# hpc4cmb/flacarray

Hardware: AMD Instinct MI355X
Metric: Msamples/s encode+decode, 4096ch x 1Msamp int32 (higher is better)
Workload: dtype int32

## Files before the change

### flacarray_amd/csrc/encode_fused.hpp

```cpp
#pragma once
#include "encode_kernels.hpp"
#include "quantize_kernels.hpp"

namespace fa {

constexpr int kFSmpWords = 65 * 32;
#ifndef FA_F_SCANW
#define FA_F_SCANW 4
#endif
#ifndef FA_F_RING
#define FA_F_RING 1024
#endif
constexpr int kFRingWords = FA_F_RING;
constexpr int kFRingMask = kFRingWords - 1;
constexpr int kFRingBlocks = kFRingWords / 64;
constexpr int kFRowBlocks = 12;
static_assert(kFRingBlocks - kFRowBlocks - 1 >= 1, "the ring must hold the longest row and a partial block beside what waits to be flushed");
constexpr int kFWaveWords = kFSmpWords + kFRingWords + 4 + 16;
constexpr int kFWaves = 4;
constexpr int kFCrcSlice = 1024;
constexpr int kFCrcXpow = 520;
#ifndef FA_F_SLEEP
#define FA_F_SLEEP 8
#endif
#ifndef FA_F_WBATCH
#define FA_F_WBATCH 4
#endif
#ifndef FA_F_CEIL
#define FA_F_CEIL 1
#endif
#ifndef FA_F_BFLY_N
#define FA_F_BFLY_N 1
#endif
#ifndef FA_F_PARKN
#define FA_F_PARKN 32
#endif
#ifndef FA_F_PARKBLK
#define FA_F_PARKBLK 1
#endif
#ifndef FA_F_PARK
#define FA_F_PARK 1
#endif
#ifndef FA_F_WAVES
#define FA_F_WAVES 3
#endif
constexpr uint32_t kLbSpinLimit = 1u << 22;

struct FusedArgs {
    const int32_t* data;
    const float* f_offsets;
    const float* f_gains;
    int64_t n_stream, stream_size, nframes, total_frames;
    int32_t max_lpc_order, max_porder, precision, pmax_full;
    int32_t tail_bs;
    double escale_full;
    const float* win;
    const uint4* hdr;
    uint8_t* blob;
    int64_t capacity;
    int64_t hb;
    uint32_t* frame_bytes;
    int64_t* frame_abs;
    FrameInfo* info;
    uint32_t* ticket;
    uint32_t* size_pub;
    unsigned long long* off_pub;
    int64_t* total;
    int* err;
    const uint16_t* crc_tab;
    unsigned long long* stamps;
    int64_t* starts;
    int64_t* nbytes;
};

__device__ __forceinline__ int fsmp_unit(int c1, int u) { return 32 * c1 + 4 * (u ^ (c1 & 7)); }
__device__ __forceinline__ int fsmp_idx(int s) {
    const int c1 = (s >> 5) + 1;
    return fsmp_unit(c1, (s >> 2) & 7) + (s & 3);
}

__device__ __forceinline__ int lane_id_opaque() {
    int l;
    asm volatile("v_mbcnt_lo_u32_b32 %0, -1, 0\n\tv_mbcnt_hi_u32_b32 %0, -1, %0" : "=v"(l));
    return l;
}
__device__ __forceinline__ int rice_fold(int r) { return (int)(((uint32_t)r << 1) ^ (uint32_t)(r >> 31)); }
__device__ __forceinline__ int dpp_wave_shr1(int old, int v) { return __builtin_amdgcn_update_dpp(old, v, 0x138, 0xF, 0xF, false); }

__device__ __forceinline__ uint16_t crc16_mulmod(uint16_t a, uint16_t b) {
    uint32_t r = 0;
#pragma unroll
    for (int i = 15; i >= 0; --i) {
        r = (r << 1) ^ ((r & 0x8000u) ? 0x18005u : 0u);
        if ((b >> i) & 1) r ^= a;
    }
    return (uint16_t)r;
}

template <typename T>
__device__ __forceinline__ T lb_load(const T* p) { return __hip_atomic_load(p, __ATOMIC_RELAXED, __HIP_MEMORY_SCOPE_AGENT); }

struct SplitRiceSearch {
    int pred_order, pmax, lane;
    uint32_t TA, TB, S, n, pb, SC, best;
    int M, p, k, bpo, kb;
    bool slot;
    __device__ __forceinline__ void start(uint32_t ta, uint32_t tb, int pred_order_, int pmax_, int lane_) {
        pred_order = pred_order_; pmax = pmax_; lane = lane_;
        TA = wave_incl_scan_u32(ta);
        TB = wave_incl_scan_u32(tb);
    }
    __device__ __forceinline__ void gather() {
        M = (2 << pmax) - 1;
        const int Lp = M - lane;
        slot = (Lp >= 1);
        const int po = slot ? (31 - __clz(Lp)) : 0;
        p = lane - (M + 1 - (2 << po));
        const uint32_t psz = 4096u >> po;
        const int cpp = 128 >> po;
        const bool inB = (po > 0) && (p >= (1 << (po - 1)));
        const int ph = inB ? (p - (1 << (po - 1))) : p;
        int hi_l = (po == 0) ? 63 : ((ph + 1) * cpp - 1);
        int lo_l = (po == 0) ? -1 : (ph * cpp - 1);
        hi_l &= 63;
        const int lo_c = lo_l < 0 ? 0 : (lo_l & 63);
        const uint32_t ah = (uint32_t)__builtin_amdgcn_ds_bpermute(hi_l << 2, (int)TA);
        const uint32_t bh = (uint32_t)__builtin_amdgcn_ds_bpermute(hi_l << 2, (int)TB);
// ... 160 lines not shown
    const int32_t* src = a.data + (s * a.stream_size + f * (int64_t)bs);
    float q_off = 0.0f, q_gain = 0.0f;
    if constexpr (F32IN) { q_off = a.f_offsets[s]; q_gain = a.f_gains[s]; }
    auto load_row = [&](int j) __attribute__((always_inline)) {
        const int4 v = reinterpret_cast<const int4*>(src)[64 * j + lane];
        if constexpr (F32IN)
            return make_int4(quantise_f32(__int_as_float(v.x), q_off, q_gain), quantise_f32(__int_as_float(v.y), q_off, q_gain),
                             quantise_f32(__int_as_float(v.z), q_off, q_gain), quantise_f32(__int_as_float(v.w), q_off, q_gain));
        else
            return v;
    };
    const float* win = a.win;
    const uint4 fhe = a.hdr[f];
    const uint32_t fh_bits = 32u + ((fhe.w >> 8) & 0xFFu) + ((fhe.w >> 16) & 0xFFu) + (fhe.w >> 24) + 8u;

#define FA_IMAGE_ADDRS                                                                  \
    const int ln_ = lane_id_opaque();                                                   \
    const int K = fsmp_unit(ln_ + 1, 0);                                                \
    const int rowbase = fsmp_unit((ln_ >> 3) + 1, ln_ & 7);                             \
    const int hist7 = fsmp_unit(ln_, 7), hist6 = fsmp_unit(ln_, 6), hist5 = fsmp_unit(ln_, 5); \
    (void)K; (void)rowbase; (void)hist7; (void)hist6; (void)hist5
    constexpr int tailA7 = 32 * 64 + 4 * (7 ^ (64 & 7)), tailA6 = 32 * 64 + 4 * (6 ^ (64 & 7)), tailA5 = 32 * 64 + 4 * (5 ^ (64 & 7));

    FA_STAMP_INIT;
#ifdef FA_TIMELINE
    const uint32_t tl_start_ = (uint32_t)__builtin_amdgcn_s_memrealtime();
#endif
    int4 Bv[8];
    uint32_t orv = 0;
    int mn, mx;
    {
        FA_IMAGE_ADDRS;
        int4 hi[8], lo[8];
#pragma unroll
        for (int j = 0; j < 8; ++j) hi[j] = load_row(8 + j);
#pragma unroll
        for (int j = 0; j < 8; ++j) lo[j] = load_row(j);
        if (lane < 32) smp[lane] = 0;
        mn = hi[0].x;
        mx = hi[0].x;
#pragma unroll
        for (int j = 0; j < 8; ++j) {
            orv |= (uint32_t)(hi[j].x | hi[j].y | hi[j].z | hi[j].w);
            mn = min(min(mn, hi[j].x), hi[j].y);
            mn = min(min(mn, hi[j].z), hi[j].w);
            mx = max(max(mx, hi[j].x), hi[j].y);
            mx = max(max(mx, hi[j].z), hi[j].w);
            *reinterpret_cast<int4*>(&smp[rowbase + 256 * j]) = hi[j];
        }
#pragma unroll
        for (int t = 0; t < 8; ++t) Bv[t] = *reinterpret_cast<const int4*>(&smp[K ^ (4 * t)]);
#pragma unroll
        for (int j = 0; j < 8; ++j) {
            orv |= (uint32_t)(lo[j].x | lo[j].y | lo[j].z | lo[j].w);
            mn = min(min(mn, lo[j].x), lo[j].y);
            mn = min(min(mn, lo[j].z), lo[j].w);
            mx = max(max(mx, lo[j].x), lo[j].y);
            mx = max(max(mx, lo[j].z), lo[j].w);
            *reinterpret_cast<int4*>(&smp[rowbase + 256 * j]) = lo[j];
        }
    }
    mn = wave_min_i32(mn);
    mx = wave_max_i32(mx);
    const bool is_const = (mn == mx);
    orv = wave_or_u32(orv);
    const int wasted = orv ? (__ffs((int)orv) - 1) : 0;
    const int bps = 32 - wasted;
    if (__builtin_expect(wasted != 0, 0)) {
        FA_IMAGE_ADDRS;
#pragma unroll
        for (int t = 0; t < 8; ++t) {
            Bv[t].x >>= wasted; Bv[t].y >>= wasted; Bv[t].z >>= wasted; Bv[t].w >>= wasted;
            int4* p = reinterpret_cast<int4*>(&smp[K ^ (4 * t)]);
            int4 v = *p;
            v.x >>= wasted; v.y >>= wasted; v.z >>= wasted; v.w >>= wasted;
            *p = v;
        }
        mn >>= wasted;
        mx >>= wasted;
    }
    const bool narrow = (mn >= -(1 << 24)) && (mx < (1 << 24));
    lds_fence();

    FA_STAMP(0);
    const uint64_t verbatim_bits = 8 + (uint64_t)wasted + (uint64_t)bs * (uint64_t)bps;
    int type = 1;
    int order = 0, porder = 0, shift = 0, precision = 0;
    int kbest = 0;
    bool img_is_residual = false;
    bool win_small_l = false, win_small_f = false;
    int fo = -1;
    int32_t qkeep[MLO];
#pragma unroll
    for (int j = 0; j < MLO; ++j) qkeep[j] = 0;
    const int pmax_geo = a.pmax_full;
    auto pmax_for = [&](int pred_order) __attribute__((always_inline)) {
        int pm = pmax_geo;
        while (pm > 0 && (bs >> pm) <= pred_order) pm--;
        return pm;
    };

    auto hist_b = [&](const int4& own, const int4& tail) __attribute__((always_inline)) {
        int4 h;
        h.x = dpp_wave_shr1(tail.x, own.x);
        h.y = dpp_wave_shr1(tail.y, own.y);
        h.z = dpp_wave_shr1(tail.z, own.z);
        h.w = dpp_wave_shr1(tail.w, own.w);
        return h;
    };

    if (__builtin_expect(is_const, 0)) {
        type = 0;
    } else {
        uint64_t best_bits = verbatim_bits;
        double tot0 = 0.0, tot1 = 0.0, tot2 = 0.0, tot3 = 0.0, tot4 = 0.0;
        double mx0 = 0.0, mx1 = 0.0, mx2 = 0.0, mx3 = 0.0, mx4 = 0.0;
        uint64_t hA0 = 0, hA1 = 0, hA2 = 0, hA3 = 0, hA4 = 0;
        double dA0 = 0.0, dA1 = 0.0, dA2 = 0.0, dA3 = 0.0, dA4 = 0.0;
        if (__builtin_expect(narrow, 1)) {
            FA_IMAGE_ADDRS;
            const uint32_t BIAS = 0x80000000u;
            uint32_t s0 = 0, s1 = 0, s2 = 0, s3 = 0, s4 = 0;
            int p1, pe1, pe2, pe3;
            auto seed = [&](const int4& hh) __attribute__((always_inline)) {
                p1 = hh.w;
                pe1 = hh.w - hh.z;
                pe2 = pe1 - (hh.z - hh.y);
                pe3 = pe2 - ((hh.z - hh.y) - (hh.y - hh.x));
            };
            auto group = [&](auto mask_tag, const int4& xv, int gi0) __attribute__((always_inline)) {
                constexpr bool MASK = decltype(mask_tag)::value;
                const int xs[4] = {xv.x, xv.y, xv.z, xv.w};
#pragma unroll
                for (int e = 0; e < 4; ++e) {
                    const int x = xs[e];
                    const int e1 = x - p1, e2 = e1 - pe1, e3 = e2 - pe2;
                    const uint32_t xb = (uint32_t)x ^ BIAS;
                    const uint32_t n0 = sad_u32(xb, BIAS, s0);
                    const uint32_t n1 = sad_u32(xb, (uint32_t)p1 ^ BIAS, s1);
                    const uint32_t n2 = sad_u32((uint32_t)e1 ^ BIAS, (uint32_t)pe1 ^ BIAS, s2);
                    const uint32_t n3 = sad_u32((uint32_t)e2 ^ BIAS, (uint32_t)pe2 ^ BIAS, s3);
                    const uint32_t n4 = sad_u32((uint32_t)e3 ^ BIAS, (uint32_t)pe3 ^ BIAS, s4);
                    if constexpr (MASK) {
                        const int gi = gi0 + e;
                        s0 = n0;
                        s1 = (gi >= 1) ? n1 : s1;
                        s2 = (gi >= 2) ? n2 : s2;
                        s3 = (gi >= 3) ? n3 : s3;
                        s4 = (gi >= 4) ? n4 : s4;
                    } else {
                        s0 = n0; s1 = n1; s2 = n2; s3 = n3; s4 = n4;
                    }
                    p1 = x; pe1 = e1; pe2 = e2; pe3 = e3;
                }
            };
            uint64_t a0 = 0, a1 = 0, a2 = 0, a3 = 0, a4 = 0;
            auto fold = [&]() __attribute__((always_inline)) {
                a0 += s0; a1 += s1; a2 += s2; a3 += s3; a4 += s4;
                s0 = s1 = s2 = s3 = s4 = 0;
            };
            seed(*reinterpret_cast<const int4*>(&smp[hist7]));
            group(std::true_type{}, *reinterpret_cast<const int4*>(&smp[K]), 32 * lane);
#pragma unroll
            for (int t = 1; t < 4; ++t) group(std::false_type{}, *reinterpret_cast<const int4*>(&smp[K ^ (4 * t)]), 0);
            fold();
#pragma unroll
            for (int t = 4; t < 8; ++t) group(std::false_type{}, *reinterpret_cast<const int4*>(&smp[K ^ (4 * t)]), 0);
            fold();
            hA0 = a0; hA1 = a1; hA2 = a2; hA3 = a3; hA4 = a4;
            seed(hist_b(Bv[7], *reinterpret_cast<const int4*>(&smp[tailA7])));
#pragma unroll
            for (int t = 0; t < 4; ++t) group(std::false_type{}, Bv[t], 0);
            fold();
#pragma unroll
            for (int t = 4; t < 8; ++t) group(std::false_type{}, Bv[t], 0);
            fold();
            tot0 = (double)a0; tot1 = (double)a1; tot2 = (double)a2; tot3 = (double)a3; tot4 = (double)a4;
        } else {
            FA_IMAGE_ADDRS;
            double p1, pe1, pe2, pe3;
            auto seed = [&](const int4& h) __attribute__((always_inline)) {
                p1 = (double)h.w;
                pe1 = (double)h.w - (double)h.z;
                const double e1b = (double)h.z - (double)h.y;
                pe2 = pe1 - e1b;
                const double e2b = e1b - ((double)h.y - (double)h.x);
                pe3 = pe2 - e2b;
            };
            auto group = [&](const int4& xv, int gi0) __attribute__((always_inline)) {
                const int xs[4] = {xv.x, xv.y, xv.z, xv.w};
#pragma unroll
                for (int e = 0; e < 4; ++e) {
                    const int gi = gi0 + e;
                    const double xd = (double)xs[e];
                    const double e1 = xd - p1;
                    const double e2 = e1 - pe1;
                    const double e3 = e2 - pe2;
                    const double e4 = e3 - pe3;
                    const double a0 = fa_fabs(xd);
                    const double a1 = (gi >= 1) ? fa_fabs(e1) : 0.0;
                    const double a2 = (gi >= 2) ? fa_fabs(e2) : 0.0;
                    const double a3 = (gi >= 3) ? fa_fabs(e3) : 0.0;
                    const double a4 = (gi >= 4) ? fa_fabs(e4) : 0.0;
                    tot0 += a0; tot1 += a1; tot2 += a2; tot3 += a3; tot4 += a4;
                    mx0 = __builtin_fmax(mx0, a0);
                    mx1 = __builtin_fmax(mx1, a1);
                    mx2 = __builtin_fmax(mx2, a2);
                    mx3 = __builtin_fmax(mx3, a3);
                    mx4 = __builtin_fmax(mx4, a4);
                    p1 = xd; pe1 = e1; pe2 = e2; pe3 = e3;
                }
            };
            seed(*reinterpret_cast<const int4*>(&smp[hist7]));
#pragma unroll 1
            for (int t = 0; t < 8; ++t) group(*reinterpret_cast<const int4*>(&smp[K ^ (4 * t)]), 32 * lane + 4 * t);
            dA0 = tot0; dA1 = tot1; dA2 = tot2; dA3 = tot3; dA4 = tot4;
            seed(hist_b(Bv[7], *reinterpret_cast<const int4*>(&smp[tailA7])));
#pragma unroll
            for (int t = 0; t < 8; ++t) group(Bv[t], 4096);
        }
        FA_STAMP(1);
        {
            double tsum[5] = {tot0, tot1, tot2, tot3, tot4};
            wave_sum_butterfly_n<5>(tsum);
            const double T0 = tsum[0], T1 = tsum[1], T2 = tsum[2], T3 = tsum[3], T4 = tsum[4];
            double M0 = 0.0, M1 = 0.0, M2 = 0.0, M3 = 0.0, M4 = 0.0;
            if (!narrow) {
                M0 = wave_max_f64(mx0); M1 = wave_max_f64(mx1); M2 = wave_max_f64(mx2); M3 = wave_max_f64(mx3);
                M4 = wave_max_f64(mx4);
            }
            const double lim = 2147483647.0;
            double smallest = 1.8446744073709552e19;
            if (M0 <= lim && T0 < smallest) { fo = 0; smallest = T0; }
            if (M1 <= lim && T1 < smallest) { fo = 1; smallest = T1; }
            if (M2 <= lim && T2 < smallest) { fo = 2; smallest = T2; }
            if (M3 <= lim && T3 < smallest) { fo = 3; smallest = T3; }
            if (M4 <= lim && T4 < smallest) { fo = 4; smallest = T4; }
        }
        uint64_t fixA, fixB;
        if (narrow) {
            const uint64_t tA = (fo == 0) ? hA0 : (fo == 1) ? hA1 : (fo == 2) ? hA2 : (fo == 3) ? hA3 : hA4;
            const double tt = (fo == 0) ? tot0 : (fo == 1) ? tot1 : (fo == 2) ? tot2 : (fo == 3) ? tot3 : tot4;
            fixA = tA;
            fixB = (uint64_t)tt - tA;
        } else {
            const double tA = (fo == 0) ? dA0 : (fo == 1) ? dA1 : (fo == 2) ? dA2 : (fo == 3) ? dA3 : dA4;
            const double tt = (fo == 0) ? tot0 : (fo == 1) ? tot1 : (fo == 2) ? tot2 : (fo == 3) ? tot3 : tot4;
            fixA = (uint64_t)tA;
            fixB = (uint64_t)(tt - tA);
        }
        int po_fix = 0, k_fix = 0;
        const int pmax_fix = pmax_for(fo < 0 ? 0 : fo);
        const bool small_fix = __all((fixA < (1u << 24)) && (fixB < (1u << 24)));
        win_small_f = small_fix;
        const bool fuse_search = fo >= 0 && pmax_fix <= 5 && a.max_lpc_order > 0 && small_fix;
        uint64_t est_fix = 0;
        auto apply_fixed = [&]() __attribute__((always_inline)) {
            if (est_fix < best_bits) {
                best_bits = est_fix;
                type = 2;
                order = fo;
                porder = po_fix;
                kbest = k_fix;
            }
        };
        if (__builtin_expect(fo >= 0 && !fuse_search, 0)) {
            uint64_t rb;
            if (pmax_fix <= 5 && small_fix) {
                SplitRiceSearch fs;
                fs.start((uint32_t)fixA, (uint32_t)fixB, fo, pmax_fix, lane);
                fs.gather(); fs.params(); fs.totals();
#pragma unroll
                for (int o = 5; o >= 0; --o) fs.order(o);
                po_fix = fs.bpo; k_fix = fs.kb; rb = fs.best;
            } else {
                rb = split_rice_search_slow(fixA, fixB, fo, pmax_fix, lane, &po_fix, &k_fix);
            }
            est_fix = 8 + (uint64_t)wasted + (uint64_t)fo * (uint64_t)bps + rb;
            apply_fixed();
        }

        FA_STAMP(2);
        int mlo = a.max_lpc_order;
        if (__builtin_expect(mlo > 0, 1)) {
            FA_IMAGE_ADDRS;
            double acc[MLO + 1];
#pragma unroll
            for (int j = 0; j <= MLO; ++j) acc[j] = 0.0;
            SplitRiceSearch fs;
            if (fuse_search) fs.start((uint32_t)fixA, (uint32_t)fixB, fo, pmax_fix, lane);
            double hist[MLO];
            struct WinV { double w[4]; };
            auto load_win = [&](int i0) __attribute__((always_inline)) {
                const float4 f = *reinterpret_cast<const float4*>(win + i0);
                WinV v;
                v.w[0] = (double)f.x; v.w[1] = (double)f.y; v.w[2] = (double)f.z; v.w[3] = (double)f.w;
                return v;
            };
            auto lag_group = [&](const int4& xv, const WinV& wv) __attribute__((always_inline)) {
                const int xs[4] = {xv.x, xv.y, xv.z, xv.w};
#pragma unroll
                for (int e = 0; e < 4; ++e) {
                    const double d = (double)xs[e] * wv.w[e];
                    acc[0] = __builtin_fma(d, d, acc[0]);
#pragma unroll
                    for (int j = 0; j < MLO; ++j) acc[j + 1] = __builtin_fma(d, hist[j], acc[j + 1]);
#pragma unroll
                    for (int j = MLO - 1; j > 0; --j) hist[j] = hist[j - 1];
                    hist[0] = d;
                }
            };
            auto search_stage = [&](int tt) __attribute__((always_inline)) {
                if (!fuse_search) return;
                if (tt == 1) fs.gather();
                if (tt == 3) fs.params();
                if (tt == 5) fs.totals();
                if (tt >= 7 && tt <= 12) fs.order(12 - tt);
            };
#if FA_F_PARK
            {
                int4* const pk = reinterpret_cast<int4*>(ring) + lane;
#pragma unroll
                for (int t = 0; t < 4; ++t) pk[64 * t] = Bv[4 + t];
            }
#endif
            {
                const int g0 = 32 * lane;
                const int4 h7 = *reinterpret_cast<const int4*>(&smp[hist7]), h6 = *reinterpret_cast<const int4*>(&smp[hist6]);
                const int4 h5 = *reinterpret_cast<const int4*>(&smp[hist5]);
                const int hs[12] = {h7.w, h7.z, h7.y, h7.x, h6.w, h6.z, h6.y, h6.x, h5.w, h5.z, h5.y, h5.x};
#pragma unroll
                for (int j = 0; j < MLO; ++j) {
                    const float wh = (g0 - 1 - j >= 0) ? win[g0 - 1 - j] : 0.0f;
                    hist[j] = (double)hs[j] * (double)wh;
                }
#pragma unroll
                for (int tb = 0; tb < 8; tb += FA_F_WBATCH) {
                    WinV wv[FA_F_WBATCH];
#pragma unroll
                    for (int t = 0; t < FA_F_WBATCH; ++t) wv[t] = load_win(g0 + 4 * (tb + t));
#pragma unroll
                    for (int t = 0; t < FA_F_WBATCH; ++t) {
                        lag_group(*reinterpret_cast<const int4*>(&smp[K ^ (4 * (tb + t))]), wv[t]);
                        search_stage(tb + t);
                    }
                    __builtin_amdgcn_sched_barrier(0);
                }
            }
#if FA_F_PARK
            {
                uint32_t pin = 16u * (uint32_t)lane;
                asm volatile("" : "+v"(pin) : "v"(__double2loint(acc[MLO])));
                const int4* const pk = reinterpret_cast<const int4*>(reinterpret_cast<const char*>(ring) + pin);
#pragma unroll
                for (int t = 0; t < 4; ++t) Bv[4 + t] = pk[64 * t];
            }
#endif
            {
                const int g0 = 2048 + 32 * lane;
                const int4 h7 = hist_b(Bv[7], *reinterpret_cast<const int4*>(&smp[tailA7]));
                const int4 h6 = hist_b(Bv[6], *reinterpret_cast<const int4*>(&smp[tailA6]));
                int4 h5 = make_int4(0, 0, 0, 0);
                if constexpr (MLO > 8) h5 = hist_b(Bv[5], *reinterpret_cast<const int4*>(&smp[tailA5]));
                const int hs[12] = {h7.w, h7.z, h7.y, h7.x, h6.w, h6.z, h6.y, h6.x, h5.w, h5.z, h5.y, h5.x};
#pragma unroll
                for (int j = 0; j < MLO; ++j) hist[j] = (double)hs[j] * (double)win[g0 - 1 - j];
#pragma unroll
                for (int tb = 0; tb < 8; tb += FA_F_WBATCH) {
                    WinV wv[FA_F_WBATCH];
#pragma unroll
                    for (int t = 0; t < FA_F_WBATCH; ++t) wv[t] = load_win(g0 + 4 * (tb + t));
#pragma unroll
                    for (int t = 0; t < FA_F_WBATCH; ++t) {
                        lag_group(Bv[tb + t], wv[t]);
                        search_stage(8 + tb + t);
                    }
                    __builtin_amdgcn_sched_barrier(0);
                }
            }
            FA_STAMP(4);
            if (fuse_search) {
                po_fix = fs.bpo;
                k_fix = fs.kb;
                est_fix = 8 + (uint64_t)wasted + (uint64_t)fo * (uint64_t)bps + (uint64_t)fs.best;
                apply_fixed();
            }
            double autoc[MLO + 1];
#if FA_F_BFLY_N
#pragma unroll
            for (int j = 0; j <= MLO; ++j) autoc[j] = acc[j];
            wave_sum_butterfly_n<MLO + 1>(autoc);
#else
#pragma unroll
            for (int j = 0; j <= MLO; ++j) autoc[j] = wave_sum_butterfly(acc[j]);
#endif

            FA_STAMP(5);
            if (__builtin_expect(autoc[0] != 0.0, 1)) {
                float* coef = reinterpret_cast<float*>(scr);
                double* err = reinterpret_cast<double*>(scr + 160);
                int* meta = reinterpret_cast<int*>(scr + 220);
                if (lane == 0) meta[0] = levinson<MLO>(autoc, mlo, coef, err);
                lds_fence();
                const int usable = meta[0];
                int prec = a.precision;
                int lo;
                {
                    double mybits = 1e300;
                    if (lane < usable) {
                        const double e = err[lane];
                        const double error_scale = a.escale_full;
                        double bpsv;
                        if (e > 0.0) {
                            bpsv = 0.5 * det_log2(error_scale * e);
                            if (!(bpsv >= 0.0)) bpsv = 0.0;
                        } else if (e < 0.0) {
                            bpsv = 1e32;
                        } else {
                            bpsv = 0.0;
                        }
                        mybits = bpsv * (double)(bs - (lane + 1)) + (double)((lane + 1) * (bps + prec));
                    }
                    double bestb = 4294967295.0;
                    int bi = 0;
#pragma unroll
                    for (int o = 0; o < MLO; ++o) {
                        const double b = readlane_f64(mybits, o);
                        if (o < usable && b < bestb) { bestb = b; bi = o; }
                    }
                    lo = bi + 1;
                }
                if (bps <= 17) {
                    const int limp = 32 - bps - ilog2_u64((uint64_t)lo);
                    if (prec > limp) prec = limp;
                }
                int sh = 0;
                int32_t qreg[MLO];
#pragma unroll
                for (int j = 0; j < MLO; ++j) qreg[j] = 0;
                int ok = 0;
                if (prec >= 2) ok = (quantize_coefs_t<MLO>(coef + (lo - 1) * MLO, lo, prec, qreg, &sh) == 0) ? 1 : 0;
                ok = __builtin_amdgcn_readfirstlane(ok);
                sh = __builtin_amdgcn_readfirstlane(sh);
#pragma unroll
                for (int j = 0; j < MLO; ++j) qreg[j] = __builtin_amdgcn_readfirstlane(qreg[j]);
                FA_STAMP(6);
                if (__builtin_expect(ok != 0, 1)) {
                    FA_IMAGE_ADDRS;
                    const double scale = bitsd((uint64_t)(1023 - sh) << 52);
                    double qd[MLO];
#pragma unroll
                    for (int j = 0; j < MLO; ++j) qd[j] = (double)qreg[j] * scale;
                    double tlA = 0.0, tlB = 0.0;
                    double hx[MLO];
                    const int4 a7 = *reinterpret_cast<const int4*>(&smp[hist7]), a6 = *reinterpret_cast<const int4*>(&smp[hist6]);
                    const int4 a5 = *reinterpret_cast<const int4*>(&smp[hist5]);
                    const int4 b7 = hist_b(Bv[7], *reinterpret_cast<const int4*>(&smp[tailA7]));
                    const int4 b6 = hist_b(Bv[6], *reinterpret_cast<const int4*>(&smp[tailA6]));
                    int4 b5 = make_int4(0, 0, 0, 0);
                    if constexpr (MLO > 8) b5 = hist_b(Bv[5], *reinterpret_cast<const int4*>(&smp[tailA5]));
                    lds_fence();
                    auto fold_f64 = [&](double r) __attribute__((always_inline)) {
                        return (int)(uint32_t)__builtin_fabs(__builtin_fma(r, 2.0, 0.5));
                    };
                    auto res_group = [&](auto mask_tag, const int4& xv, int gi0, double& tl) __attribute__((always_inline)) {
                        constexpr bool MASK = decltype(mask_tag)::value;
                        const int xs[4] = {xv.x, xv.y, xv.z, xv.w};
                        int rs[4];
#pragma unroll
                        for (int e = 0; e < 4; ++e) {
                            const double xd = (double)xs[e];
#if FA_F_CEIL
                            double t = xd;
#pragma unroll
                            for (int j = 0; j < MLO; ++j) t = __builtin_fma(-qd[j], hx[j], t);
                            const double r = fa_ceil(t);
#else
                            double sum = 0.0;
#pragma unroll
                            for (int j = 0; j < MLO; ++j) sum = __builtin_fma(qd[j], hx[j], sum);
                            const double pred = fa_floor(sum);
                            const double r = xd - pred;
#endif
                            if constexpr (MASK) {
                                const bool v = (gi0 + e >= lo);
                                tl += v ? fa_fabs(r) : 0.0;
                                rs[e] = v ? fold_f64(r) : xs[e];
                            } else {
                                tl += fa_fabs(r);
                                rs[e] = fold_f64(r);
                            }
#pragma unroll
                            for (int j = MLO - 1; j > 0; --j) hx[j] = hx[j - 1];
                            hx[0] = xd;
                        }
                        return make_int4(rs[0], rs[1], rs[2], rs[3]);
                    };
                    constexpr int kWarmGroups = (MLO + 3) / 4;
                    {
                        const int hs[12] = {a7.w, a7.z, a7.y, a7.x, a6.w, a6.z, a6.y, a6.x, a5.w, a5.z, a5.y, a5.x};
#pragma unroll
                        for (int j = 0; j < MLO; ++j) hx[j] = (double)hs[j];
#pragma unroll
                        for (int t = 0; t < 8; ++t) {
                            int4* px = reinterpret_cast<int4*>(&smp[K ^ (4 * t)]);
                            if (t < kWarmGroups) *px = res_group(std::true_type{}, *px, 32 * lane + 4 * t, tlA);
                            else *px = res_group(std::false_type{}, *px, 0, tlA);
                        }
                    }
                    {
                        const int hs[12] = {b7.w, b7.z, b7.y, b7.x, b6.w, b6.z, b6.y, b6.x, b5.w, b5.z, b5.y, b5.x};
#pragma unroll
                        for (int j = 0; j < MLO; ++j) hx[j] = (double)hs[j];
#pragma unroll
                        for (int t = 0; t < 8; ++t) Bv[t] = res_group(std::false_type{}, Bv[t], 0, tlB);
                    }
                    FA_STAMP(7);
                    img_is_residual = true;
                    const int pmax = pmax_for(lo);
                    int po_l = 0, k_l = 0;
                    uint64_t rbits;
                    const bool small_l = __all((tlA < 16777216.0) && (tlB < 16777216.0));
                    bool lpc_in_range = true;
                    if (__builtin_expect(!small_l, 0)) {
                        bool hit = false;
#pragma unroll 1
                        for (int t = 0; t < 8; ++t) {
                            const int4 ra = *reinterpret_cast<const int4*>(&smp[K ^ (4 * t)]);
                            const int ras[4] = {ra.x, ra.y, ra.z, ra.w};
#pragma unroll
                            for (int e = 0; e < 4; ++e) hit = hit || ((32 * lane + 4 * t + e >= lo) && (uint32_t)ras[e] == 0xffffffffu);
                        }
#pragma unroll
                        for (int t = 0; t < 8; ++t)
                            hit = hit || (uint32_t)Bv[t].x == 0xffffffffu || (uint32_t)Bv[t].y == 0xffffffffu || (uint32_t)Bv[t].z == 0xffffffffu ||
                                  (uint32_t)Bv[t].w == 0xffffffffu;
                        lpc_in_range = !__any(hit);
                    }
                    win_small_l = small_l;
                    if (pmax <= 5 && small_l) {
                        SplitRiceSearch ls;
                        ls.start((uint32_t)tlA, (uint32_t)tlB, lo, pmax, lane);
                        ls.gather(); ls.params(); ls.totals();
#pragma unroll
                        for (int o = 5; o >= 0; --o) ls.order(o);
                        po_l = ls.bpo; k_l = ls.kb; rbits = ls.best;
                    } else {
                        rbits = split_rice_search_slow((uint64_t)tlA, (uint64_t)tlB, lo, pmax, lane, &po_l, &k_l);
                    }
                    if (lpc_in_range) {
                        const uint64_t est = 8 + (uint64_t)wasted + 4 + 5 + (uint64_t)lo * (uint64_t)(prec + bps) + rbits;
                        if (est < best_bits) {
                            best_bits = est;
                            type = 3;
                            order = lo;
                            porder = po_l;
                            kbest = k_l;
                            shift = sh;
                            precision = prec;
#pragma unroll
                            for (int j = 0; j < MLO; ++j) qkeep[j] = qreg[j];
                        }
                    }
                }
                lds_fence();
            }
        }
    }

    FA_STAMP(8);
    const int lane_w = lane_id_opaque();
    auto reload_image = [&]() __attribute__((always_inline)) {
        FA_IMAGE_ADDRS;
#pragma unroll 1
        for (int half = 1; half >= 0; --half) {
#pragma unroll
            for (int j = 0; j < 8; ++j) {
                int4 v = load_row(8 * half + j);
                v.x >>= wasted; v.y >>= wasted; v.z >>= wasted; v.w >>= wasted;
                *reinterpret_cast<int4*>(&smp[rowbase + 256 * j]) = v;
            }
            if (half == 1) {
#pragma unroll
                for (int t = 0; t < 8; ++t) Bv[t] = *reinterpret_cast<const int4*>(&smp[K ^ (4 * t)]);
            }
        }
        lds_fence();
    };
    if (__builtin_expect(type == 2, 0)) {
        if (img_is_residual) {
            reload_image();
            img_is_residual = false;
        }
        {
            FA_IMAGE_ADDRS;
            const int4 ha = *reinterpret_cast<const int4*>(&smp[hist7]);
            const int4 hb2 = hist_b(Bv[7], *reinterpret_cast<const int4*>(&smp[tailA7]));
            lds_fence();
            int64_t x1, x2, x3, x4;
            auto fgroup = [&](const int4& xv, int gi0) __attribute__((always_inline)) {
                const int xs[4] = {xv.x, xv.y, xv.z, xv.w};
                int rs[4];
#pragma unroll
                for (int e = 0; e < 4; ++e) {
                    const int64_t x0 = xs[e];
                    int64_t r;
                    if (order == 0) r = x0;
                    else if (order == 1) r = x0 - x1;
                    else if (order == 2) r = x0 - 2 * x1 + x2;
                    else if (order == 3) r = x0 - 3 * x1 + 3 * x2 - x3;
                    else r = x0 - 4 * x1 + 6 * x2 - 4 * x3 + x4;
                    rs[e] = (gi0 + e >= order) ? rice_fold((int)r) : xs[e];
                    x4 = x3; x3 = x2; x2 = x1; x1 = x0;
                }
                return make_int4(rs[0], rs[1], rs[2], rs[3]);
            };
            x1 = ha.w; x2 = ha.z; x3 = ha.y; x4 = ha.x;
#pragma unroll 1
            for (int t = 0; t < 8; ++t) {
                int4* px = reinterpret_cast<int4*>(&smp[K ^ (4 * t)]);
                *px = fgroup(*px, 32 * lane_w + 4 * t);
            }
            x1 = hb2.w; x2 = hb2.z; x3 = hb2.y; x4 = hb2.x;
#pragma unroll
            for (int t = 0; t < 8; ++t) Bv[t] = fgroup(Bv[t], 4096);
            img_is_residual = true;
        }
        lds_fence();
    }

    bool rice2 = false;
    if (type >= 2) rice2 = __any((lane_w < (1 << porder)) && (kbest >= 15));
    const int plen = rice2 ? 5 : 4;
    uint32_t sub_bits;
    if (type >= 2) {
        FA_IMAGE_ADDRS;
        const int pA = (lane_w << porder) >> 7, pB = ((64 + lane_w) << porder) >> 7;
        const uint32_t kA = (uint32_t)__builtin_amdgcn_ds_bpermute(pA << 2, kbest);
        const uint32_t kB = (uint32_t)__builtin_amdgcn_ds_bpermute(pB << 2, kbest);
        const uint32_t cpp = 128u >> porder;
        uint32_t bitsA = 0, bitsB = 0;
        auto size_group = [&](auto mask_tag, auto clamp_tag, const int4& rv, uint32_t k, int gi0, uint32_t& acc) __attribute__((always_inline)) {
            constexpr bool MASK = decltype(mask_tag)::value;
            constexpr bool CLAMP = decltype(clamp_tag)::value;
            const int rs[4] = {rv.x, rv.y, rv.z, rv.w};
#pragma unroll
            for (int e = 0; e < 4; ++e) {
                const uint32_t u = (uint32_t)rs[e];
                uint32_t q = u >> k;
                if constexpr (CLAMP) q = min(q, 16384u);
                if constexpr (MASK) q = (gi0 + e >= order) ? (q + k + 1u) : 0u;
                acc += q;
            }
        };
        constexpr int kWarmGroupsS = (MLO + 3) / 4 > 1 ? (MLO + 3) / 4 : 1;
        auto size_lane = [&](auto clamp_tag) __attribute__((always_inline)) {
#pragma unroll
            for (int t = 0; t < 8; ++t) {
                const int4 rv = *reinterpret_cast<const int4*>(&smp[K ^ (4 * t)]);
                if (t < kWarmGroupsS) size_group(std::true_type{}, clamp_tag, rv, kA, 32 * lane_w + 4 * t, bitsA);
                else size_group(std::false_type{}, clamp_tag, rv, kA, 0, bitsA);
            }
#pragma unroll
            for (int t = 0; t < 8; ++t) size_group(std::false_type{}, clamp_tag, Bv[t], kB, 0, bitsB);
        };
        if (__builtin_expect((type == 3) ? win_small_l : win_small_f, 1)) size_lane(std::false_type{});
        else size_lane(std::true_type{});
        bitsA += (8 - kWarmGroupsS) * 4 * (kA + 1u);
        bitsB += 32u * (kB + 1u);
        if (((uint32_t)lane_w & (cpp - 1u)) == 0u || cpp > 64u) {
            if (cpp <= 64u) { bitsA += (uint32_t)plen; bitsB += (uint32_t)plen; }
            else if (lane_w == 0) bitsA += (uint32_t)plen;
        }
        uint32_t rA = bitsA, rB = bitsB;
        rA += (uint32_t)xchg_i32<0>((int)rA); rB += (uint32_t)xchg_i32<0>((int)rB);
        rA += (uint32_t)xchg_i32<1>((int)rA); rB += (uint32_t)xchg_i32<1>((int)rB);
        rA += (uint32_t)xchg_i32<2>((int)rA); rB += (uint32_t)xchg_i32<2>((int)rB);
        const bool row_over = __any((rA > (uint32_t)kRowCapBits) || (rB > (uint32_t)kRowCapBits));
        const uint64_t exact = 6 + wave_sum_u64((uint64_t)bitsA + bitsB) + 8 + (uint64_t)wasted + (uint64_t)order * (uint64_t)bps +
                               ((type == 3) ? (4 + 5 + (uint64_t)order * (uint64_t)precision) : 0);
        if (row_over || exact > verbatim_bits) {
            type = 1;
            order = 0;
            porder = 0;
        }
        sub_bits = (uint32_t)exact;
    }
    if (type == 0) sub_bits = 8u + (uint32_t)wasted + (uint32_t)bps;
    if (type == 1) sub_bits = (uint32_t)verbatim_bits;
    const uint32_t total_bytes = ((fh_bits + sub_bits + 7u) >> 3) + 2u;
    const uint32_t L = total_bytes - 2u;

    FA_STAMP(9);
    const uint32_t F = (uint32_t)a.total_frames;
    const uint32_t gu = (uint32_t)g;
#ifdef FA_TIMELINE
    if (lane_w == 0 && a.info) {
        a.info[g].wasted = (int32_t)tl_start_;
        a.info[g].shift = (int32_t)(uint32_t)__builtin_amdgcn_s_memrealtime();
        __builtin_amdgcn_s_waitcnt(0);
    }
#endif
    if (lane_w == 0) {
        __hip_atomic_store(a.size_pub + gu, 0x80000000u | total_bytes, __ATOMIC_RELAXED, __HIP_MEMORY_SCOPE_AGENT);
        a.frame_bytes[g] = total_bytes;
    }
    (void)F;
#ifndef FA_TIMELINE
    if (lane_w == 0 && a.info) {
        FrameInfo fi;
        fi.type = type;
        fi.order = (type >= 2) ? order : 0;
        fi.porder = (type >= 2) ? porder : 0;
        fi.wasted = wasted;
        fi.shift = (type == 3) ? shift : 0;
        fi.precision = (type == 3) ? precision : 0;
        fi.nbytes = (int32_t)total_bytes;
        fi.blocksize = bs;
        a.info[g] = fi;
    }
#endif

#ifdef FA_F_ANALYSIS_ONLY
    if (lane_w == 0) a.frame_abs[g] = g * (int64_t)kSlotBytes + (s + 1) * a.hb;
    return;
#endif
    kpar[lane_w] = (uint8_t)kbest;
    for (int i = lane_w; i < kFRingWords; i += 64) ring[i] = 0;
    if (lane_w == 0) ring[kFRingWords] = 0;
    lds_fence();
    uint32_t pos = 0;
    uint32_t blocks_flushed = 0;
    uint8_t* dst = nullptr;
    bool dropped = false, have_dst = false;
    uint32_t crc_t = 0;

    auto put_bits = [&](uint32_t P, uint32_t val, uint32_t nb) __attribute__((always_inline)) {
        const uint32_t off = P & 31u;
        const uint64_t X = (uint64_t)val << (64u - nb - off);
        const uint32_t a0 = (P >> 3) & (uint32_t)(4 * kFRingWords - 4);
        atomicOr(reinterpret_cast<uint32_t*>(reinterpret_cast<char*>(ring) + a0), (uint32_t)(X >> 32));
        atomicOr(reinterpret_cast<uint32_t*>(reinterpret_cast<char*>(ring) + a0 + 4), (uint32_t)X);
    };
    auto put_code = [&](uint32_t P, uint32_t u, uint32_t shl) __attribute__((always_inline)) {
        const uint32_t vL = (u << shl) | 0x80000000u;
        uint32_t wi;
        asm("v_bfe_u32 %0, %1, 5, %2" : "=v"(wi) : "v"(P), "n"(__builtin_ctz((unsigned)kFRingWords)));
        uint32_t* const w = ring + wi;
        atomicOr(w, __builtin_amdgcn_alignbit(0u, vL, P));
        atomicOr(w + 1, __builtin_amdgcn_alignbit(vL, 0u, P));
    };
    unsigned long long off_word = 0;
    auto lb_issue = [&]() __attribute__((always_inline)) {
#ifndef FA_F_NOLB
        off_word = lb_load(a.off_pub + gu);
#endif
    };
    auto lb_resolve = [&]() __attribute__((always_inline)) {
        uint32_t spins = 0;
        bool fail = false;
#ifdef FA_TIMELINE
        const uint32_t tl_req_ = (uint32_t)__builtin_amdgcn_s_memrealtime();
#endif
#ifdef FA_F_NOLB
        off_word = (unsigned long long)(g * (int64_t)kSlotBytes + (s + 1) * a.hb);
#else
        while (off_word == 0) {
            __builtin_amdgcn_s_sleep(FA_F_SLEEP);
            if (++spins > kLbSpinLimit) { fail = true; break; }
            off_word = lb_load(a.off_pub + gu);
        }
#endif
#ifdef FA_TIMELINE
        if (lane_w == 0 && a.info) {
            a.info[g].precision = (int32_t)tl_req_;
            a.info[g].blocksize = (int32_t)(uint32_t)__builtin_amdgcn_s_memrealtime();
// ... 441 lines not shown
```

### flacarray_amd/csrc/encode_kernels.hpp

```cpp
#pragma once
#include <hip/hip_runtime.h>
#include <stdint.h>

#include <type_traits>

#include "flac_math.hpp"

namespace fa {

#ifndef FA_UNIT_COMPACT

struct FrameInfo {
    int32_t type, order, porder, wasted, shift, precision, nbytes, blocksize;
};

struct EncodeArgs {
    const int32_t* data;
    int64_t n_stream;
    int64_t stream_size;
    int64_t nframes;
    int32_t B;
    int32_t tail_bs;
    int32_t max_lpc_order;
    int32_t max_porder;
// ... 52 lines not shown
        st_[k] += t_ - t_prev_;                                  \
        t_prev_ = fa_memtime();                                  \
    } while (0)
#define FA_STAMP_INIT                 \
    unsigned long long st_[16];       \
    for (int i_ = 0; i_ < 16; ++i_) st_[i_] = 0; \
    unsigned long long t_prev_ = fa_memtime()
#define FA_STAMP_FLUSH                                                                   \
    do {                                                                                 \
        if (threadIdx.x == 0 && a.stamps && (blockIdx.x & 63) == 0) {                    \
            for (int i_ = 0; i_ < 16; ++i_) atomicAdd(&a.stamps[i_], st_[i_]);           \
            atomicAdd(&a.stamps[16], 1ULL);                                              \
        }                                                                                \
    } while (0)
#elif defined(FA_PHASE_MARKS)
#define FA_STAMP(k)                                   \
    do {                                              \
        __builtin_amdgcn_sched_barrier(0);            \
        asm volatile("; FA_MARK " #k ::: "memory");   \
        __builtin_amdgcn_sched_barrier(0);            \
    } while (0)
#define FA_STAMP_INIT FA_STAMP(init)
#define FA_STAMP_FLUSH FA_STAMP(end)
#else
#define FA_STAMP(k) do { } while (0)
#define FA_STAMP_INIT do { } while (0)
#define FA_STAMP_FLUSH do { } while (0)
#endif

constexpr int kChunkStride = 68;
constexpr int kSmpWords = 65 * kChunkStride;
constexpr int kRingWords = 512;
constexpr int kRingMask = kRingWords - 1;
constexpr int kLdsWords = kSmpWords + kRingWords + 2 + 128 + 16;

__device__ __forceinline__ int smp_idx(int s) { return kChunkStride * ((s >> 6) + 1) + (s & 63); }

__device__ __forceinline__ void lds_fence() { asm volatile("s_waitcnt lgkmcnt(0)" ::: "memory"); }

template <int CTRL>
__device__ __forceinline__ int dpp_i32(int v) {
    return __builtin_amdgcn_update_dpp(0, v, CTRL, 0xF, 0xF, true);
}
constexpr int kDppXor1 = 0xB1;
constexpr int kDppXor2 = 0x4E;
constexpr int kDppHalfMirror = 0x141;
constexpr int kDppMirror = 0x140;
constexpr int kSwzXor16 = 0x401F;

template <int STEP>
__device__ __forceinline__ int xchg_i32(int v) {
    if constexpr (STEP == 0) return dpp_i32<kDppXor1>(v);
    else if constexpr (STEP == 1) return dpp_i32<kDppXor2>(v);
    else if constexpr (STEP == 2) return dpp_i32<kDppHalfMirror>(v);
    else if constexpr (STEP == 3) return dpp_i32<kDppMirror>(v);
    else return __builtin_amdgcn_ds_swizzle(v, kSwzXor16);
}
template <int STEP>
__device__ __forceinline__ double xchg_f64(double v) {
    const int lo = xchg_i32<STEP>(__double2loint(v)), hi = xchg_i32<STEP>(__double2hiint(v));
    return __hiloint2double(hi, lo);
}
template <int STEP>
__device__ __forceinline__ uint64_t xchg_u64(uint64_t v) {
    const uint32_t lo = (uint32_t)xchg_i32<STEP>((int)(uint32_t)v), hi = (uint32_t)xchg_i32<STEP>((int)(uint32_t)(v >> 32));
    return ((uint64_t)hi << 32) | lo;
}
__device__ __forceinline__ double readlane_f64(double v, int l) {
    return __hiloint2double(__builtin_amdgcn_readlane(__double2hiint(v), l), __builtin_amdgcn_readlane(__double2loint(v), l));
}
__device__ __forceinline__ uint64_t readlane_u64(uint64_t v, int l) {
    return ((uint64_t)(uint32_t)__builtin_amdgcn_readlane((int)(uint32_t)(v >> 32), l) << 32) |
           (uint32_t)__builtin_amdgcn_readlane((int)(uint32_t)v, l);
}

__device__ __forceinline__ double wave_sum_butterfly(double v) {
    v = v + xchg_f64<0>(v);
    v = v + xchg_f64<1>(v);
    v = v + xchg_f64<2>(v);
    v = v + xchg_f64<3>(v);
    v = v + xchg_f64<4>(v);
    return readlane_f64(v, 0) + readlane_f64(v, 32);
}
template <int N>
__device__ __forceinline__ void wave_sum_butterfly_n(double (&v)[N]) {
    double o[N];
#define FA_BF_STEP(S)                                          \
    _Pragma("unroll") for (int i = 0; i < N; ++i) o[i] = xchg_f64<S>(v[i]); \
    _Pragma("unroll") for (int i = 0; i < N; ++i) v[i] = v[i] + o[i];
    FA_BF_STEP(0)
    FA_BF_STEP(1)
    FA_BF_STEP(2)
    FA_BF_STEP(3)
    FA_BF_STEP(4)
#undef FA_BF_STEP
#pragma unroll
    for (int i = 0; i < N; ++i) v[i] = readlane_f64(v[i], 0) + readlane_f64(v[i], 32);
}
__device__ __forceinline__ double wave_max_f64(double v) {
    double o;
    o = xchg_f64<0>(v); v = (o > v) ? o : v;
    o = xchg_f64<1>(v); v = (o > v) ? o : v;
    o = xchg_f64<2>(v); v = (o > v) ? o : v;
    o = xchg_f64<3>(v); v = (o > v) ? o : v;
    o = xchg_f64<4>(v); v = (o > v) ? o : v;
    const double a = readlane_f64(v, 0), b = readlane_f64(v, 32);
    return (b > a) ? b : a;
}
__device__ __forceinline__ uint64_t wave_sum_u64(uint64_t v) {
    v += xchg_u64<0>(v);
    v += xchg_u64<1>(v);
    v += xchg_u64<2>(v);
    v += xchg_u64<3>(v);
    v += xchg_u64<4>(v);
    return readlane_u64(v, 0) + readlane_u64(v, 32);
}
__device__ __forceinline__ uint32_t wave_or_u32(uint32_t v) {
    v |= (uint32_t)xchg_i32<0>((int)v);
    v |= (uint32_t)xchg_i32<1>((int)v);
    v |= (uint32_t)xchg_i32<2>((int)v);
    v |= (uint32_t)xchg_i32<3>((int)v);
    v |= (uint32_t)xchg_i32<4>((int)v);
    return (uint32_t)__builtin_amdgcn_readlane((int)v, 0) | (uint32_t)__builtin_amdgcn_readlane((int)v, 32);
}
__device__ __forceinline__ int wave_min_i32(int v) {
    v = min(v, xchg_i32<0>(v));
    v = min(v, xchg_i32<1>(v));
    v = min(v, xchg_i32<2>(v));
    v = min(v, xchg_i32<3>(v));
    v = min(v, xchg_i32<4>(v));
    return min(__builtin_amdgcn_readlane(v, 0), __builtin_amdgcn_readlane(v, 32));
}
__device__ __forceinline__ int wave_max_i32(int v) {
    v = max(v, xchg_i32<0>(v));
    v = max(v, xchg_i32<1>(v));
    v = max(v, xchg_i32<2>(v));
    v = max(v, xchg_i32<3>(v));
    v = max(v, xchg_i32<4>(v));
    return max(__builtin_amdgcn_readlane(v, 0), __builtin_amdgcn_readlane(v, 32));
}
__device__ __forceinline__ uint32_t wave_incl_scan_u32(uint32_t v) {
    v += (uint32_t)__builtin_amdgcn_update_dpp(0, (int)v, 0x111, 0xF, 0xF, true);
    v += (uint32_t)__builtin_amdgcn_update_dpp(0, (int)v, 0x112, 0xF, 0xF, true);
    v += (uint32_t)__builtin_amdgcn_update_dpp(0, (int)v, 0x114, 0xF, 0xF, true);
    v += (uint32_t)__builtin_amdgcn_update_dpp(0, (int)v, 0x118, 0xF, 0xF, true);
    v += (uint32_t)__builtin_amdgcn_update_dpp(0, (int)v, 0x142, 0xA, 0xF, false);
    v += (uint32_t)__builtin_amdgcn_update_dpp(0, (int)v, 0x143, 0xC, 0xF, false);
    return v;
}

__device__ __forceinline__ uint32_t sad_u32(uint32_t a, uint32_t b, uint32_t c) {
    uint32_t r;
    asm("v_sad_u32 %0, %1, %2, %3" : "=v"(r) : "v"(a), "v"(b), "v"(c));
    return r;
}

__device__ __forceinline__ void ring_put(uint32_t* ring, uint32_t pos, uint32_t v, int n) {
    uint32_t w = pos >> 5;
    int off = (int)(pos & 31);
    uint64_t t = (((uint64_t)v) << (64 - n)) >> off;
    uint32_t hi = (uint32_t)(t >> 32), lo = (uint32_t)t;
    if (hi) atomicOr(&ring[w & kRingMask], hi);
    if (lo) atomicOr(&ring[(w + 1) & kRingMask], lo);
}

__device__ __forceinline__ uint64_t wave_incl_scan_u64(uint64_t v) {
#define FA_SCAN_STEP(CTRL, RM, BC)                                                                         \
    {                                                                                                      \
        const uint32_t lo_ = (uint32_t)__builtin_amdgcn_update_dpp(0, (int)(uint32_t)v, CTRL, RM, 0xF, BC);        \
        const uint32_t hi_ = (uint32_t)__builtin_amdgcn_update_dpp(0, (int)(uint32_t)(v >> 32), CTRL, RM, 0xF, BC); \
        v += ((uint64_t)hi_ << 32) | lo_;                                                                  \
    }
    FA_SCAN_STEP(0x111, 0xF, true)
    FA_SCAN_STEP(0x112, 0xF, true)
    FA_SCAN_STEP(0x114, 0xF, true)
    FA_SCAN_STEP(0x118, 0xF, true)
    FA_SCAN_STEP(0x142, 0xA, false)
    FA_SCAN_STEP(0x143, 0xC, false)
#undef FA_SCAN_STEP
    return v;
}
__device__ __forceinline__ uint64_t gather_u64(uint64_t v, int src_lane) {
    const uint32_t lo = (uint32_t)__builtin_amdgcn_ds_bpermute(src_lane << 2, (int)(uint32_t)v);
    const uint32_t hi = (uint32_t)__builtin_amdgcn_ds_bpermute(src_lane << 2, (int)(uint32_t)(v >> 32));
    return ((uint64_t)hi << 32) | lo;
}

__device__ __forceinline__ void rice_search_batch(uint64_t T, int bs, int pred_order, int po_hi, int po_lo, int lane,
                                                  bool* have, uint64_t* best, int* best_po, int* kbest) {
    const int M = (2 << po_hi) - 1;
    const int Lp = M - lane;
    const int po = (Lp >= 1) ? (31 - __clz(Lp)) : 0;
    const bool slot = (Lp >= 1) && (po >= po_lo);
    const int p = lane - (M + 1 - (2 << po));
    const uint32_t psz = (uint32_t)(bs >> po);
    const int lpp = (po == 0) ? 64 : (int)(psz / kChunk);
    int hi_l = (p + 1) * lpp - 1, lo_l = p * lpp - 1;
    hi_l = hi_l > 63 ? 63 : (hi_l < 0 ? 0 : hi_l);
// ... 1343 lines not shown
```

Before: 204,200.

## Use integer wave reductions for narrow sums and halve multi-value butterfly traffic

For narrow frames, the fixed-predictor residual sums are reduced as 32-bit integers when every lane's totals fit under 2^26, falling back to 64-bit integer sums otherwise. This replaces five double-precision butterfly reductions with cheaper integer lane exchanges. The generic N-value double butterfly is rewritten as a recursive-halving scheme in which each lane keeps half its slots and exchanges the other half per step, so fewer cross-lane exchanges are issued, with results read from computed owner lanes. A compile-time FA_F_STOP_AT early-exit probe is also added; it is inactive by default.

```diff
diff --git a/flacarray_amd/csrc/encode_fused.hpp b/flacarray_amd/csrc/encode_fused.hpp
--- a/flacarray_amd/csrc/encode_fused.hpp
+++ b/flacarray_amd/csrc/encode_fused.hpp
@@ -43,6 +43,35 @@
 #endif
 #ifndef FA_F_WAVES
 #define FA_F_WAVES 3
+#endif
+#ifdef FA_F_STOP_AT
+__device__ __forceinline__ void fa_sink(int v) { asm volatile("" ::"v"(v)); }
+__device__ __forceinline__ void fa_sink(uint32_t v) { asm volatile("" ::"v"(v)); }
+__device__ __forceinline__ void fa_sink(uint64_t v) { asm volatile("" ::"v"(v)); }
+__device__ __forceinline__ void fa_sink(double v) { asm volatile("" ::"v"(v)); }
+__device__ __forceinline__ void fa_sink(bool v) { fa_sink((int)v); }
+__device__ __forceinline__ void fa_sink(const int4& v) { fa_sink(v.x); fa_sink(v.y); fa_sink(v.z); fa_sink(v.w); }
+template <typename T, int N>
+__device__ __forceinline__ void fa_sink(const T (&v)[N]) {
+#pragma unroll
+    for (int i = 0; i < N; ++i) fa_sink(v[i]);
+}
+template <typename... T>
+__device__ __forceinline__ void fa_sinks(const T&... v) { (fa_sink(v), ...); }
+#define FA_F_STOP(k, cond, ...)                                                                                \
+    do {                                                                                                       \
+        if ((cond) || FA_F_STOP_AT == (k)) {                                                                   \
+            fa_sinks(Bv, mn, mx, orv __VA_OPT__(,) __VA_ARGS__);                                               \
+            if (lane == 0) {                                                                                   \
+                __hip_atomic_store(a.size_pub + (uint32_t)g, 0x80000000u, __ATOMIC_RELAXED, __HIP_MEMORY_SCOPE_AGENT); \
+                a.frame_bytes[g] = 0u;                                                                         \
+                a.frame_abs[g] = (s + 1) * a.hb;                                                               \
+            }                                                                                                  \
+            return;                                                                                            \
+        }                                                                                                      \
+    } while (0)
+#else
+#define FA_F_STOP(k, cond, ...) do { } while (0)
 #endif
 constexpr uint32_t kLbSpinLimit = 1u << 22;
 
@@ -369,7 +398,7 @@
     const bool narrow = (mn >= -(1 << 24)) && (mx < (1 << 24));
     lds_fence();
 
-    FA_STAMP(0);
+    FA_STAMP(0); FA_F_STOP(0, false);
     const uint64_t verbatim_bits = 8 + (uint64_t)wasted + (uint64_t)bs * (uint64_t)bps;
     int type = 1;
     int order = 0, porder = 0, shift = 0, precision = 0;
@@ -403,6 +432,7 @@
         double tot0 = 0.0, tot1 = 0.0, tot2 = 0.0, tot3 = 0.0, tot4 = 0.0;
         double mx0 = 0.0, mx1 = 0.0, mx2 = 0.0, mx3 = 0.0, mx4 = 0.0;
         uint64_t hA0 = 0, hA1 = 0, hA2 = 0, hA3 = 0, hA4 = 0;
+        uint64_t u0 = 0, u1 = 0, u2 = 0, u3 = 0, u4 = 0;
         double dA0 = 0.0, dA1 = 0.0, dA2 = 0.0, dA3 = 0.0, dA4 = 0.0;
         if (__builtin_expect(narrow, 1)) {
             FA_IMAGE_ADDRS;
@@ -463,6 +493,7 @@
             for (int t = 4; t < 8; ++t) group(std::false_type{}, Bv[t], 0);
             fold();
             tot0 = (double)a0; tot1 = (double)a1; tot2 = (double)a2; tot3 = (double)a3; tot4 = (double)a4;
+            u0 = a0; u1 = a1; u2 = a2; u3 = a3; u4 = a4;
         } else {
             FA_IMAGE_ADDRS;
             double p1, pe1, pe2, pe3;
@@ -506,10 +537,21 @@
 #pragma unroll
             for (int t = 0; t < 8; ++t) group(Bv[t], 4096);
         }
-        FA_STAMP(1);
+        FA_STAMP(1); FA_F_STOP(1, false, tot0, tot1, tot2, tot3, tot4, hA0, hA1, hA2, hA3, hA4, u0, u1, u2, u3, u4, dA0, mx0, mx4);
         {
             double tsum[5] = {tot0, tot1, tot2, tot3, tot4};
-            wave_sum_butterfly_n<5>(tsum);
+            if (__builtin_expect(narrow, 1)) {
+                if (__builtin_expect(__all((u0 | u1 | u2 | u3 | u4) < (1ull << 26)), 1)) {
+                    tsum[0] = (double)wave_sum_u32((uint32_t)u0); tsum[1] = (double)wave_sum_u32((uint32_t)u1);
+                    tsum[2] = (double)wave_sum_u32((uint32_t)u2); tsum[3] = (double)wave_sum_u32((uint32_t)u3);
+                    tsum[4] = (double)wave_sum_u32((uint32_t)u4);
+                } else {
+                    tsum[0] = (double)wave_sum_u64(u0); tsum[1] = (double)wave_sum_u64(u1); tsum[2] = (double)wave_sum_u64(u2);
+                    tsum[3] = (double)wave_sum_u64(u3); tsum[4] = (double)wave_sum_u64(u4);
+                }
+            } else {
+                wave_sum_butterfly_n<5>(tsum);
+            }
             const double T0 = tsum[0], T1 = tsum[1], T2 = tsum[2], T3 = tsum[3], T4 = tsum[4];
             double M0 = 0.0, M1 = 0.0, M2 = 0.0, M3 = 0.0, M4 = 0.0;
             if (!narrow) {
@@ -567,7 +609,7 @@
             apply_fixed();
         }
 
-        FA_STAMP(2);
+        FA_STAMP(2); FA_F_STOP(2, false, fo, fixA, fixB, fuse_search, best_bits, type, order, porder, kbest);
         int mlo = a.max_lpc_order;
         if (__builtin_expect(mlo > 0, 1)) {
             FA_IMAGE_ADDRS;
@@ -665,7 +707,7 @@
                     __builtin_amdgcn_sched_barrier(0);
                 }
             }
-            FA_STAMP(4);
+            FA_STAMP(4); FA_F_STOP(4, false, acc, fs.best, fs.bpo, fs.kb, best_bits, fo, fixA, fixB);
             if (fuse_search) {
                 po_fix = fs.bpo;
                 k_fix = fs.kb;
@@ -682,7 +724,7 @@
             for (int j = 0; j <= MLO; ++j) autoc[j] = wave_sum_butterfly(acc[j]);
 #endif
 
-            FA_STAMP(5);
+            FA_STAMP(5); FA_F_STOP(5, false, autoc, best_bits, type, order, porder, kbest);
             if (__builtin_expect(autoc[0] != 0.0, 1)) {
                 float* coef = reinterpret_cast<float*>(scr);
                 double* err = reinterpret_cast<double*>(scr + 160);
@@ -731,7 +773,7 @@
                 sh = __builtin_amdgcn_readfirstlane(sh);
 #pragma unroll
                 for (int j = 0; j < MLO; ++j) qreg[j] = __builtin_amdgcn_readfirstlane(qreg[j]);
-                FA_STAMP(6);
+                FA_STAMP(6); FA_F_STOP(6, false, qreg, sh, ok, lo, prec, best_bits, type, order, porder, kbest);
                 if (__builtin_expect(ok != 0, 1)) {
                     FA_IMAGE_ADDRS;
                     const double scale = bitsd((uint64_t)(1023 - sh) << 52);
@@ -802,7 +844,7 @@
 #pragma unroll
                         for (int t = 0; t < 8; ++t) Bv[t] = res_group(std::false_type{}, Bv[t], 0, tlB);
                     }
-                    FA_STAMP(7);
+                    FA_STAMP(7); FA_F_STOP(7, false, tlA, tlB, lo, prec, sh, qreg, best_bits, type, order, porder, kbest);
                     img_is_residual = true;
                     const int pmax = pmax_for(lo);
                     int po_l = 0, k_l = 0;
@@ -855,7 +897,7 @@
         }
     }
 
-    FA_STAMP(8);
+    FA_STAMP(8); FA_F_STOP(8, FA_F_STOP_AT < 8, type, order, porder, kbest, shift, precision, qkeep, img_is_residual, win_small_l, win_small_f);
     const int lane_w = lane_id_opaque();
     auto reload_image = [&]() __attribute__((always_inline)) {
         FA_IMAGE_ADDRS;
@@ -978,7 +1020,7 @@
     const uint32_t total_bytes = ((fh_bits + sub_bits + 7u) >> 3) + 2u;
     const uint32_t L = total_bytes - 2u;
 
-    FA_STAMP(9);
+    FA_STAMP(9); FA_F_STOP(9, false, total_bytes, type, order, porder, kbest, shift, precision, qkeep, rice2);
     const uint32_t F = (uint32_t)a.total_frames;
     const uint32_t gu = (uint32_t)g;
 #ifdef FA_TIMELINE
diff --git a/flacarray_amd/csrc/encode_kernels.hpp b/flacarray_amd/csrc/encode_kernels.hpp
--- a/flacarray_amd/csrc/encode_kernels.hpp
+++ b/flacarray_amd/csrc/encode_kernels.hpp
@@ -158,20 +158,78 @@
     v = v + xchg_f64<4>(v);
     return readlane_f64(v, 0) + readlane_f64(v, 32);
 }
+__host__ __device__ constexpr int bfly_choice(int step, int l) {
+    return step == 0 ? ((l ^ (l >> 2)) & 1)
+         : step == 1 ? (((l >> 1) ^ (l >> 2)) & 1)
+         : step == 2 ? (((l >> 2) ^ (l >> 3)) & 1)
+         : step == 3 ? ((l >> 3) & 1)
+                     : ((l >> 4) & 1);
+}
+__host__ __device__ constexpr uint32_t bfly_choice_mask(int step) {
+    uint32_t m = 0;
+    for (int l = 0; l < 32; ++l) m |= (uint32_t)bfly_choice(step, l) << l;
+    return m;
+}
+__host__ __device__ constexpr int bfly_open(int N, int step) {
+    int n = N;
+    for (int k = 0; k < step; ++k) n = n / 2 + (n & 1);
+    return n;
+}
+__host__ __device__ constexpr int bfly_owner(int N, int i) {
+    for (int l = 0; l < 32; ++l) {
+        int slot = i;
+        bool held = true;
+        for (int k = 0; k < 5 && held; ++k) {
+            const int n = bfly_open(N, k), P = n / 2;
+            if (slot < 2 * P) {
+                const int want = (slot >= P) ? 1 : 0;
+                held = bfly_choice(k, l) == want;
+                slot -= want * P;
+            } else {
+                slot = P;
+            }
+        }
+        if (held) return l;
+    }
+    return -1;
+}
+template <int N>
+struct BflyOwners {
+    int l[N];
+    constexpr BflyOwners() : l() {
+        for (int i = 0; i < N; ++i) l[i] = bfly_owner(N, i);
+    }
+};
 template <int N>
 __device__ __forceinline__ void wave_sum_butterfly_n(double (&v)[N]) {
-    double o[N];
-#define FA_BF_STEP(S)                                          \
-    _Pragma("unroll") for (int i = 0; i < N; ++i) o[i] = xchg_f64<S>(v[i]); \
-    _Pragma("unroll") for (int i = 0; i < N; ++i) v[i] = v[i] + o[i];
+    static_assert(N >= 1 && N <= 32 && bfly_open(N, 5) == 1, "one slot per lane after five halvings");
+    const uint32_t lane = __builtin_amdgcn_mbcnt_hi(~0u, __builtin_amdgcn_mbcnt_lo(~0u, 0u));
+    double w[N];
+#pragma unroll
+    for (int i = 0; i < N; ++i) w[i] = v[i];
+#define FA_BF_STEP(S)                                                                           \
+    {                                                                                           \
+        constexpr int n = bfly_open(N, S), P = n / 2, M = P + (n & 1);                          \
+        const bool c = ((bfly_choice_mask(S) >> (lane & 31u)) & 1u) != 0u;                     \
+        double snd[M];                                                                          \
+        _Pragma("unroll") for (int j = 0; j < P; ++j) {                                         \
+            snd[j] = c ? w[j] : w[j + P];                                                       \
+            w[j] = c ? w[j + P] : w[j];                                                         \
+        }                                                                                       \
+        if constexpr ((n & 1) != 0) w[P] = w[2 * P];                                            \
+        if constexpr ((n & 1) != 0) snd[P] = w[P];                                              \
+        _Pragma("unroll") for (int j = 0; j < M; ++j) snd[j] = xchg_f64<S>(snd[j]);             \
+        _Pragma("unroll") for (int j = 0; j < M; ++j) w[j] = w[j] + snd[j];                     \
+    }
     FA_BF_STEP(0)
     FA_BF_STEP(1)
     FA_BF_STEP(2)
     FA_BF_STEP(3)
     FA_BF_STEP(4)
 #undef FA_BF_STEP
-#pragma unroll
-    for (int i = 0; i < N; ++i) v[i] = readlane_f64(v[i], 0) + readlane_f64(v[i], 32);
+    constexpr BflyOwners<N> own{};
+#pragma unroll
+    for (int i = 0; i < N; ++i) v[i] = readlane_f64(w[0], own.l[i]) + readlane_f64(w[0], own.l[i] + 32);
 }
 __device__ __forceinline__ double wave_max_f64(double v) {
     double o;
@@ -190,6 +248,14 @@
     v += xchg_u64<3>(v);
     v += xchg_u64<4>(v);
     return readlane_u64(v, 0) + readlane_u64(v, 32);
+}
+__device__ __forceinline__ uint32_t wave_sum_u32(uint32_t v) {
+    v += (uint32_t)xchg_i32<0>((int)v);
+    v += (uint32_t)xchg_i32<1>((int)v);
+    v += (uint32_t)xchg_i32<2>((int)v);
+    v += (uint32_t)xchg_i32<3>((int)v);
+    v += (uint32_t)xchg_i32<4>((int)v);
+    return (uint32_t)__builtin_amdgcn_readlane((int)v, 0) + (uint32_t)__builtin_amdgcn_readlane((int)v, 32);
 }
 __device__ __forceinline__ uint32_t wave_or_u32(uint32_t v) {
     v |= (uint32_t)xchg_i32<0>((int)v);
```

Measured after the change: 205,400, median of 6. No clear change (+0.6%).
